# Substra/substrafl

Hardware: AMD Instinct MI355X
Metric: aggregated-param GB/s (device-resident) FedAvg reduce, N clients × M params (higher is better)
Workload: dtype f32

## Files before the change

substrafl_amd/csrc/host_pool.h:

```cpp
#pragma once

#include <algorithm>
#include <atomic>
#include <condition_variable>
#include <cstdint>
#include <cstring>
#include <deque>
#include <functional>
#include <mutex>
#include <thread>
#include <vector>

#include <pthread.h>
#include <sched.h>

namespace fedagg_host {

inline bool bind_thread(const std::vector<int>& cpus) {
  if (cpus.empty()) return true;
  cpu_set_t set;
  CPU_ZERO(&set);
  for (int c : cpus)
    if (c >= 0 && c < CPU_SETSIZE) CPU_SET(c, &set);
  return pthread_setaffinity_np(pthread_self(), sizeof(set), &set) == 0;
}

class Pool {
 public:
  explicit Pool(int n, std::vector<int> cpus = {}) : cpus_(std::move(cpus)) {
    for (int i = 0; i < n; ++i) th_.emplace_back([this] { run(); });
  }
  ~Pool() {
    {
      std::lock_guard<std::mutex> g(m_);
      stop_ = true;
    }
    cv_.notify_all();
    for (auto& t : th_) t.join();
  }
  void submit(std::function<void()> f) {
    {
      std::lock_guard<std::mutex> g(m_);
      q_.push_back(std::move(f));
    }
    cv_.notify_one();
  }
  int size() const { return (int)th_.size(); }
  const std::vector<int>& cpus() const { return cpus_; }

 private:
  void run() {
    bind_thread(cpus_);
    for (;;) {
      std::function<void()> f;
      {
        std::unique_lock<std::mutex> l(m_);
        cv_.wait(l, [this] { return stop_ || !q_.empty(); });
        if (stop_ && q_.empty()) return;
        f = std::move(q_.front());
        q_.pop_front();
      }
      f();
    }
  }
  const std::vector<int> cpus_;
  std::vector<std::thread> th_;
  std::deque<std::function<void()>> q_;
  std::mutex m_;
  std::condition_variable cv_;
  bool stop_ = false;
};

struct Done {
  std::mutex m;
  std::condition_variable cv;
  bool done = false;
  void set() {
    std::lock_guard<std::mutex> g(m);
    done = true;
    cv.notify_all();
  }
  void wait() {
    std::unique_lock<std::mutex> l(m);
    cv.wait(l, [this] { return done; });
  }
};

inline void gather_range(const void* const* ptr, const uint64_t* len, int nseg, uint64_t a, uint64_t b, char* dst) {
  uint64_t off = 0;
  for (int i = 0; i < nseg && off < b; ++i) {
    const uint64_t s0 = off, s1 = off + len[i];
    off = s1;
    const uint64_t lo = std::max(a, s0), hi = std::min(b, s1);
    if (lo >= hi) continue;
    memcpy(dst + (lo - a), static_cast<const char*>(ptr[i]) + (lo - s0), hi - lo);
  }
}

template <typename T>
inline uint64_t count_value_mismatch(const char* x, const char* r, uint64_t n) {
  uint64_t bad = 0;
  for (uint64_t i = 0; i < n; ++i) {
    T a, b;
    memcpy(&a, x + i * sizeof(T), sizeof(T));
    memcpy(&b, r + i * sizeof(T), sizeof(T));
    bad += !((a == b) || (a != a && b != b));
  }
  return bad;
}

enum { kHalfNone = 0, kHalfF16 = 1, kHalfBF16 = 2 };

inline uint64_t count_value_mismatch16(const char* x, const char* r, uint64_t n, uint16_t inf_bits) {
  uint64_t bad = 0;
  for (uint64_t i = 0; i < n; ++i) {
    uint16_t a, b;
    memcpy(&a, x + i * 2, 2);
    memcpy(&b, r + i * 2, 2);
    const uint16_t ma = a & 0x7FFF, mb = b & 0x7FFF;
    bad += !((a == b) || ((ma | mb) == 0) || (ma > inf_bits && mb > inf_bits));
  }
  return bad;
}

inline uint64_t count_mismatch_range(const void* const* x, const void* const* ref, const uint64_t* len, int nseg,
                                     uint64_t a, uint64_t b, int esz, int half = kHalfNone) {
  uint64_t off = 0, bad = 0;
  for (int i = 0; i < nseg && off < b; ++i) {
    const uint64_t s0 = off, s1 = off + len[i];
    off = s1;
    const uint64_t lo = std::max(a, s0), hi = std::min(b, s1);
    if (lo >= hi) continue;
    const char* px = static_cast<const char*>(x[i]) + (lo - s0);
    const char* pr = static_cast<const char*>(ref[i]) + (lo - s0);
    if (px == pr) continue;
    for (uint64_t u = 0; u < hi - lo; u += 4096) {
      const uint64_t n = std::min<uint64_t>(4096, hi - lo - u);
      if (!memcmp(px + u, pr + u, n)) continue;
      bad += half ? count_value_mismatch16(px + u, pr + u, n / 2, half == kHalfBF16 ? 0x7F80 : 0x7C00)
             : esz == 8 ? count_value_mismatch<double>(px + u, pr + u, n / 8)
                        : count_value_mismatch<float>(px + u, pr + u, n / 4);
    }
  }
  return bad;
}

struct Ring {
  std::vector<void*> slot;
  std::vector<bool> used;
  uint64_t chunk_bytes = 0;
  int size() const { return (int)slot.size(); }
};

inline uint64_t check_rows(Pool& pool, const void* const* h_seg, const uint64_t* seg_bytes, int nseg, int K,
                           uint64_t byte_lo, uint64_t row, int esz, int half = kHalfNone) {
  const uint64_t piece = 1ull << 20;
  const uint64_t npieces = (K >= 2 && row) ? (row + piece - 1) / piece : 0;
  std::atomic<uint64_t> bad{0};
  std::vector<Done> cdone(npieces ? npieces : 1);
  for (uint64_t p = 0; p < npieces; ++p) {
    const uint64_t a = byte_lo + p * piece, b = byte_lo + std::min(row, (p + 1) * piece);
    Done* d = &cdone[p];
    pool.submit([=, &bad] {
      uint64_t n = 0;
      for (int k = 1; k < K; ++k) n += count_mismatch_range(h_seg + (size_t)k * nseg, h_seg, seg_bytes, nseg, a, b, esz, half);
      bad.fetch_add(n, std::memory_order_relaxed);
      d->set();
    });
  }
  for (uint64_t p = 0; p < npieces; ++p) cdone[p].wait();
  return bad.load();
}

template <class Eng, class Pack, class Copy>
int ring_stage(Eng& eng, Pool& pool, Ring& ring, uint64_t units, bool two_queues, Pack pack, Copy copy) {
  const int R = ring.size();
  const bool two = two_queues && units > 1;
  std::vector<Done> done(units ? std::min<uint64_t>(units, (uint64_t)R) : 1);
  std::vector<bool> pending(done.size(), false);
  int rc = 0;
  uint64_t next_submit = 0;
  auto submit = [&](uint64_t u) {
    const int slot = (int)(u % R);
    if (ring.used[slot]) eng.wait(slot);
    ring.used[slot] = false;
    Done& d = done[slot];
    d.done = false;
    pending[slot] = true;
    char* dst = static_cast<char*>(ring.slot[slot]);
    pool.submit([=, &d] {
      pack(u, dst);
      d.set();
    });
  };
  for (; next_submit < units && next_submit + 1 < (uint64_t)R; ++next_submit) submit(next_submit);
  for (uint64_t u = 0; u < units && !rc; ++u) {
    const int slot = (int)(u % R);
    done[slot].wait();
    pending[slot] = false;
    const int q = (two && (u & 1)) ? 1 : 0;
    rc = copy(u, static_cast<const char*>(ring.slot[slot]), q);
    if (!rc) rc = eng.mark(slot, q);
    if (!rc) ring.used[slot] = true;
    if (!rc && next_submit < units) submit(next_submit++);
  }
  for (size_t i = 0; i < done.size(); ++i)
    if (pending[i]) done[i].wait();
  return rc;
}

template <class Eng>
int stage_pipeline(Eng& eng, Pool& pool, Ring& ring, const void* const* h_seg, const uint64_t* seg_bytes, int nseg,
                   int K, uint64_t byte_lo, uint64_t row, char* d_dst, uint64_t ld_bytes, bool two_queues,
                   int check_esz = 0, uint64_t* mismatches = nullptr, int check_half = kHalfNone) {
  const uint64_t cb = ring.chunk_bytes;
  const int Ks = check_esz ? 1 : K;
  const uint64_t per_row = row ? (row + cb - 1) / cb : 0;
  const int rc = ring_stage(
      eng, pool, ring, per_row * (uint64_t)Ks, two_queues,
      [=](uint64_t u, char* dst) {
        const uint64_t a = (u % per_row) * cb, b = std::min(row, a + cb);
        gather_range(h_seg + (size_t)(u / per_row) * nseg, seg_bytes, nseg, byte_lo + a, byte_lo + b, dst);
      },
      [&, per_row, cb](uint64_t u, const char* slot, int q) {
        const uint64_t a = (u % per_row) * cb;
        return eng.h2d(q, d_dst + (u / per_row) * ld_bytes + a, slot, std::min(row, a + cb) - a);
      });
  if (rc || !check_esz || K < 2) return rc;
  const uint64_t bad = check_rows(pool, h_seg, seg_bytes, nseg, K, byte_lo, row, check_esz, check_half);
  if (mismatches) *mismatches += bad;
  return 0;
}

template <class Eng>
int stage_tiled_pipeline(Eng& eng, Pool& pool, Ring& ring, const void* const* h_seg, const uint64_t* seg_bytes,
                         int nseg, int K, uint64_t row, uint64_t tb, char* d_dst, bool two_queues) {
  if (!tb || tb > ring.chunk_bytes) return -1;
  const uint64_t tiles = row ? (row + tb - 1) / tb : 0;
  const uint64_t blocks = tiles * (uint64_t)K, bpu = ring.chunk_bytes / tb;
  return ring_stage(
      eng, pool, ring, (blocks + bpu - 1) / bpu, two_queues,
      [=](uint64_t u, char* dst) {
        const uint64_t j1 = std::min(blocks, (u + 1) * bpu);
        for (uint64_t j = u * bpu; j < j1; ++j) {
          const uint64_t t = j / (uint64_t)K, a = t * tb, b = std::min(row, a + tb);
          gather_range(h_seg + (size_t)(j % (uint64_t)K) * nseg, seg_bytes, nseg, a, b, dst + (j - u * bpu) * tb);
        }
      },
      [&, blocks, bpu](uint64_t u, const char* slot, int q) {
        return eng.h2d(q, d_dst + u * bpu * tb, slot, (std::min(blocks, (u + 1) * bpu) - u * bpu) * tb);
      });
}

template <class Eng>
int stage_row_tiled_pipeline(Eng& eng, Pool& pool, Ring& ring, const void* const* h_seg, const uint64_t* seg_bytes,
                             int nseg, uint64_t row, uint64_t tb, int K, int k, char* d_dst, bool two_queues) {
  if (!tb || tb > ring.chunk_bytes || K <= 0 || k < 0 || k >= K) return -1;
  const uint64_t tiles = row ? (row + tb - 1) / tb : 0, tpu = ring.chunk_bytes / tb;
  return ring_stage(
      eng, pool, ring, (tiles + tpu - 1) / tpu, two_queues,
      [=](uint64_t u, char* dst) {
        const uint64_t a = u * tpu * tb;
        gather_range(h_seg, seg_bytes, nseg, a, std::min(row, a + tpu * tb), dst);
      },
      [&, tiles, tpu](uint64_t u, const char* slot, int q) {
        const uint64_t t0 = u * tpu, n = std::min(tiles, t0 + tpu) - t0;
        return eng.h2d_2d(q, d_dst + (t0 * (uint64_t)K + (uint64_t)k) * tb, (uint64_t)K * tb, slot, tb, tb, n);
      });
}

template <class Eng>
int fetch_pipeline(Eng& eng, Pool& pool, Ring& ring, const char* d_src, char* h_dst, uint64_t bytes) {
  const uint64_t cb = ring.chunk_bytes;
  const int R = ring.size();
  const int G = std::max(1, std::min(4, R / 2));
  const int NG = R / G;
  const uint64_t sb = cb * (uint64_t)G;
  const uint64_t units = (bytes + sb - 1) / sb;
  std::vector<Done> done(R);
  std::vector<bool> pending(R, false);
  int rc = 0;
  for (uint64_t u = 0; u < units && !rc; ++u) {
    const int g0 = (int)(u % (uint64_t)NG) * G;
    for (int i = 0; i < G; ++i)
      if (pending[g0 + i]) {
        done[g0 + i].wait();
        pending[g0 + i] = false;
      }
    const uint64_t a = u * sb, b = std::min(bytes, a + sb);
    rc = eng.d2h(ring.slot[g0], d_src + a, b - a);
    if (!rc) rc = eng.mark(g0, 0);
    if (rc) break;
    for (int i = 0; i < G; ++i) ring.used[g0 + i] = i == 0;
    for (int i = 0; i < G; ++i) {
      const uint64_t pa = a + (uint64_t)i * cb;
      if (pa >= b) break;
      const uint64_t pb = std::min(b, pa + cb);
      const int slot = g0 + i;
      done[slot].done = false;
      pending[slot] = true;
      const char* src = static_cast<const char*>(ring.slot[slot]);
      char* dst = h_dst + pa;
      Done* d = &done[slot];
      pool.submit([=, &eng] {
        eng.wait(g0);
        memcpy(dst, src, pb - pa);
        d->set();
      });
    }
  }
  for (int i = 0; i < R; ++i)
    if (pending[i]) done[i].wait();
  return rc;
}

}
```

substrafl_amd/csrc/session.hip:

```cpp

#include <hip/hip_runtime.h>

#include <algorithm>
#include <atomic>
#include <chrono>
#include <condition_variable>
#include <cstdint>
#include <cstdio>
#include <cstring>
#include <deque>
#include <functional>
#include <mutex>
#include <thread>
#include <vector>

#include <sys/syscall.h>
#include <unistd.h>

#include "fedagg_internal.h"
#include "host_pool.h"

using fedagg_host::Pool;
using fedagg_host::Ring;

namespace {

int hip_fail(const char* what, hipError_t e) {
  char buf[512];
  snprintf(buf, sizeof(buf), "%s: %s", what, hipGetErrorString(e));
  fedagg_internal::set_error(buf);
  return FEDAGG_EHIP;
}

#define HIP_TRY(call)                                     \
  do {                                                    \
    hipError_t e_ = (call);                               \
    if (e_ != hipSuccess) return hip_fail(#call, e_);     \
  } while (0)

}

struct fedagg_session {
  int device = 0;
  hipStream_t stream = nullptr;
  hipStream_t xstream = nullptr;
  hipEvent_t join_ev = nullptr;
  int copy_streams = 2;
  int threads = 8;
  uint64_t chunk_bytes = 4ull << 20;
  int slots = 12;
  void* ring_base = nullptr;
  Ring ring;
  std::vector<hipEvent_t> ring_ev;
  void* dbuf[FEDAGG_SESSION_BUFFERS] = {};
  uint64_t dbytes[FEDAGG_SESSION_BUFFERS] = {};
  hipEvent_t tev[FEDAGG_SESSION_EVENTS] = {};
  Pool* pool = nullptr;
  double last_stage_s = 0, last_fetch_s = 0;
  uint64_t fail_copy_after = 0;
  uint64_t copies = 0;
  std::vector<int> cpus;
  double phase[FEDAGG_SESSION_PHASES] = {};

  int ensure_ring() {
    if (ring.size() == slots && ring.chunk_bytes == chunk_bytes) return FEDAGG_OK;
    release_ring();
    ring.slot.assign(slots, nullptr);
    ring_ev.assign(slots, nullptr);
    ring.used.assign(slots, false);
    ring.chunk_bytes = chunk_bytes;
    hipError_t e;
    if (cpus.empty()) {
      e = hipHostMalloc(&ring_base, (size_t)slots * chunk_bytes, hipHostMallocDefault);
    } else {
      e = hipErrorUnknown;
      std::thread t([&] {
        (void)hipSetDevice(device);
        if (fedagg_host::bind_thread(cpus))
          e = hipHostMalloc(&ring_base, (size_t)slots * chunk_bytes, hipHostMallocNumaUser);
        else
          e = hipHostMalloc(&ring_base, (size_t)slots * chunk_bytes, hipHostMallocDefault);
      });
      t.join();
    }
    if (e != hipSuccess) {
      ring_base = nullptr;
      release_ring();
      return hip_fail("hipHostMalloc(staging ring)", e);
    }
    for (int i = 0; i < slots; ++i) {
      ring.slot[i] = static_cast<char*>(ring_base) + (size_t)i * chunk_bytes;
      if ((e = hipEventCreateWithFlags(&ring_ev[i], hipEventDisableTiming)) != hipSuccess) {
        ring_ev[i] = nullptr;
        release_ring();
        return hip_fail("hipEventCreate(staging ring)", e);
      }
    }
    return FEDAGG_OK;
  }
  void release_ring() {
    for (size_t i = 0; i < ring_ev.size(); ++i) {
      if (ring_ev[i]) {
        (void)hipEventSynchronize(ring_ev[i]);
        (void)hipEventDestroy(ring_ev[i]);
      }
    }
    if (ring_base) (void)hipHostFree(ring_base);
    ring_base = nullptr;
    ring.slot.clear();
    ring.used.clear();
    ring.chunk_bytes = 0;
    ring_ev.clear();
  }
  std::mutex pool_m;
  Pool& workers() {
    std::lock_guard<std::mutex> g(pool_m);
    if (!pool || pool->size() != threads || pool->cpus() != cpus) {
      delete pool;
      pool = new Pool(threads, cpus);
    }
    return *pool;
  }
};

namespace {

double now_s() {
  return std::chrono::duration<double>(std::chrono::steady_clock::now().time_since_epoch()).count();
}

struct HipEngine {
  fedagg_session* s;
  bool injected() { return s->fail_copy_after && ++s->copies >= s->fail_copy_after; }
  int h2d(int q, void* d, const void* h, uint64_t n) {
    if (injected()) return hip_fail("hipMemcpyAsync(H2D) [injected by the fail_copy_after knob]", hipErrorUnknown);
    hipError_t e = hipMemcpyAsync(d, h, n, hipMemcpyHostToDevice, q ? s->xstream : s->stream);
    return e == hipSuccess ? FEDAGG_OK : hip_fail("hipMemcpyAsync(H2D)", e);
  }
  int h2d_2d(int q, void* d, uint64_t dpitch, const void* h, uint64_t spitch, uint64_t width, uint64_t height) {
    if (injected()) return hip_fail("hipMemcpy2DAsync(H2D) [injected by the fail_copy_after knob]", hipErrorUnknown);
    hipError_t e = hipMemcpy2DAsync(d, dpitch, h, spitch, width, height, hipMemcpyHostToDevice,
                                    q ? s->xstream : s->stream);
    return e == hipSuccess ? FEDAGG_OK : hip_fail("hipMemcpy2DAsync(H2D)", e);
  }
  int d2h(void* h, const void* d, uint64_t n) {
    if (injected()) return hip_fail("hipMemcpyAsync(D2H) [injected by the fail_copy_after knob]", hipErrorUnknown);
    hipError_t e = hipMemcpyAsync(h, d, n, hipMemcpyDeviceToHost, s->stream);
    return e == hipSuccess ? FEDAGG_OK : hip_fail("hipMemcpyAsync(D2H)", e);
  }
  int mark(int slot, int q) {
    hipError_t e = hipEventRecord(s->ring_ev[slot], q ? s->xstream : s->stream);
    return e == hipSuccess ? FEDAGG_OK : hip_fail("hipEventRecord(ring)", e);
  }
  void wait(int slot) { (void)hipEventSynchronize(s->ring_ev[slot]); }
};

}

extern "C" {

fedagg_session* fedagg_session_create(int device) {
  const double t0 = now_s();
  int n = 0;
  hipError_t e = hipGetDeviceCount(&n);
  if (e != hipSuccess || n <= 0) {
    hip_fail("fedagg_session_create: no HIP device", e == hipSuccess ? hipErrorNoDevice : e);
    return nullptr;
  }
  if (device < 0 || device >= n) {
    fedagg_internal::set_error("fedagg_session_create: device index out of range");
    return nullptr;
  }
  if ((e = hipSetDevice(device)) != hipSuccess) {
    hip_fail("hipSetDevice", e);
    return nullptr;
  }
  auto* s = new fedagg_session();
  s->device = device;
  const double t1 = now_s();
  s->phase[0] = t1 - t0;
  if ((e = hipStreamCreateWithFlags(&s->stream, hipStreamNonBlocking)) != hipSuccess ||
      (e = hipStreamCreateWithFlags(&s->xstream, hipStreamNonBlocking)) != hipSuccess ||
      (e = hipEventCreateWithFlags(&s->join_ev, hipEventDisableTiming)) != hipSuccess) {
    hip_fail("fedagg_session_create: stream/event", e);
    if (s->xstream) (void)hipStreamDestroy(s->xstream);
    if (s->stream) (void)hipStreamDestroy(s->stream);
    delete s;
    return nullptr;
  }
  s->phase[1] = now_s() - t1;
  return s;
}

void fedagg_session_destroy(fedagg_session* s) {
  if (!s) return;
  (void)hipSetDevice(s->device);
  (void)hipStreamSynchronize(s->stream);
  (void)hipStreamSynchronize(s->xstream);
  s->release_ring();
  for (int i = 0; i < FEDAGG_SESSION_BUFFERS; ++i)
    if (s->dbuf[i]) (void)hipFree(s->dbuf[i]);
  for (int i = 0; i < FEDAGG_SESSION_EVENTS; ++i)
    if (s->tev[i]) (void)hipEventDestroy(s->tev[i]);
  (void)hipEventDestroy(s->join_ev);
  (void)hipStreamDestroy(s->xstream);
  (void)hipStreamDestroy(s->stream);
  delete s->pool;
  delete s;
}

void* fedagg_session_stream(fedagg_session* s) { return s ? (void*)s->stream : nullptr; }

int fedagg_session_set(fedagg_session* s, const char* key, long long value) {
  if (!s || !key) return FEDAGG_EINVAL;
  if (!strcmp(key, "threads") && value >= 1 && value <= 256) {
    s->threads = (int)value;
    if (s->slots < s->threads + 2) {
      s->release_ring();
      s->slots = s->threads + 2;
    }
  } else if (!strcmp(key, "chunk_bytes") && value >= (1 << 16)) {
    s->release_ring();
    s->chunk_bytes = (uint64_t)value;
  } else if (!strcmp(key, "copy_streams") && (value == 1 || value == 2)) {
    s->copy_streams = (int)value;
  } else if (!strcmp(key, "slots") && value >= 2 && value <= 1024) {
    s->release_ring();
    s->slots = (int)std::max<long long>(value, s->threads + 1);
  } else if (!strcmp(key, "fail_copy_after") && value >= 0) {
    s->fail_copy_after = (uint64_t)value;
    s->copies = 0;
  } else {
    fedagg_internal::set_error("fedagg_session_set: unknown key or bad value");
    return FEDAGG_EINVAL;
  }
  return FEDAGG_OK;
}

int fedagg_session_affinity(fedagg_session* s, const int* cpus, int ncpus) {
  if (!s || ncpus < 0 || (ncpus && !cpus)) {
    fedagg_internal::set_error("fedagg_session_affinity: invalid argument");
    return FEDAGG_EINVAL;
  }
  std::vector<int> v(cpus, cpus + ncpus);
  for (int c : v)
    if (c < 0 || c >= CPU_SETSIZE) {
      fedagg_internal::set_error("fedagg_session_affinity: CPU index out of range");
      return FEDAGG_EINVAL;
    }
  std::lock_guard<std::mutex> g(s->pool_m);
  if (v != s->cpus) {
    int caller = -1;
    (void)hipGetDevice(&caller);
    (void)hipSetDevice(s->device);
    s->release_ring();
    s->cpus = std::move(v);
    if (caller >= 0) (void)hipSetDevice(caller);
  }
  return FEDAGG_OK;
}

int fedagg_session_ring_node(fedagg_session* s) {
  if (!s || !s->ring_base) return -1;
  int node = -1;
  if (syscall(SYS_get_mempolicy, &node, nullptr, 0UL, s->ring_base, 3UL) != 0) return -1;
  return node;
}

int fedagg_device_pci_bus_id(int device, char* buf, int len) {
  if (!buf || len < 13) {
    fedagg_internal::set_error("fedagg_device_pci_bus_id: buffer too small");
    return FEDAGG_EINVAL;
  }
  hipError_t e = hipDeviceGetPCIBusId(buf, len, device);
  return e == hipSuccess ? FEDAGG_OK : hip_fail("hipDeviceGetPCIBusId", e);
}

int fedagg_session_buffer(fedagg_session* s, int slot, uint64_t bytes, void** d_ptr) {
  if (!s || slot < 0 || slot >= FEDAGG_SESSION_BUFFERS || !d_ptr) return FEDAGG_EINVAL;
  HIP_TRY(hipSetDevice(s->device));
  if (s->dbytes[slot] < bytes) {
    if (s->dbuf[slot]) {
      HIP_TRY(hipStreamSynchronize(s->stream));
      HIP_TRY(hipFree(s->dbuf[slot]));
      s->dbuf[slot] = nullptr;
      s->dbytes[slot] = 0;
    }
    HIP_TRY(hipMalloc(&s->dbuf[slot], bytes));
    s->dbytes[slot] = bytes;
  }
  *d_ptr = s->dbuf[slot];
  return FEDAGG_OK;
}

int fedagg_session_warm(fedagg_session* s, const uint64_t* slot_bytes, int nslots) {
  if (!s || nslots < 0 || nslots > FEDAGG_SESSION_BUFFERS || (nslots > 0 && !slot_bytes)) return FEDAGG_EINVAL;
  HIP_TRY(hipSetDevice(s->device));
  double t = now_s();
  int rc = s->ensure_ring();
  if (rc) return rc;
  s->phase[2] = now_s() - t;
  t = now_s();
  (void)s->workers();
  s->phase[3] = now_s() - t;
  t = now_s();
  void* probe = nullptr;
  for (int i = 0; i < nslots; ++i) {
    if (!slot_bytes[i]) continue;
    void* d = nullptr;
    rc = fedagg_session_buffer(s, i, slot_bytes[i], &d);
    if (rc) return rc;
    if (!probe && slot_bytes[i] >= 4096) probe = d;
  }
  if (!probe) {
    rc = fedagg_session_buffer(s, FEDAGG_SESSION_BUFFERS - 1, 4096, &probe);
    if (rc) return rc;
  }
  s->phase[4] = now_s() - t;
  t = now_s();
  HIP_TRY(hipMemsetAsync(probe, 0, 4096, s->stream));
  rc = fedagg_read_probe_f32(static_cast<const float*>(probe), 512, static_cast<float*>(probe) + 512, 1,
                             (void*)s->stream);
  if (rc) return rc;
  HIP_TRY(hipStreamSynchronize(s->stream));
  s->phase[5] = now_s() - t;
  return FEDAGG_OK;
}

int fedagg_session_stage(fedagg_session* s, void* d_dst, uint64_t ld_bytes, int K, int nseg,
                         const void* const* h_seg, const uint64_t* seg_bytes) {
  if (nseg < 0 || (nseg > 0 && !seg_bytes)) return FEDAGG_EINVAL;
  uint64_t row = 0;
  for (int i = 0; i < nseg; ++i) row += seg_bytes[i];
  return fedagg_session_stage_range(s, d_dst, ld_bytes, K, nseg, h_seg, seg_bytes, 0, row);
}

namespace {

int stage_prepare(fedagg_session* s, void* d_dst, uint64_t ld_bytes, int K, int nseg, const void* const* h_seg,
                  const uint64_t* seg_bytes, uint64_t byte_lo, uint64_t byte_hi, uint64_t* row_out) {
  if (!s || !d_dst || K <= 0 || nseg < 0 || (nseg > 0 && (!h_seg || !seg_bytes)) || byte_hi < byte_lo)
    return FEDAGG_EINVAL;
  HIP_TRY(hipSetDevice(s->device));
  int rc = s->ensure_ring();
  if (rc) return rc;
  uint64_t full = 0;
  for (int i = 0; i < nseg; ++i) full += seg_bytes[i];
  if (byte_hi > full) {
    fedagg_internal::set_error("fedagg_session_stage_range: byte range beyond the row");
    return FEDAGG_EINVAL;
  }
  const uint64_t row = byte_hi - byte_lo;
  if (row > ld_bytes) {
    fedagg_internal::set_error("fedagg_session_stage: segments exceed the row stride");
    return FEDAGG_EINVAL;
  }
  for (int k = 0; k < K; ++k)
    for (int i = 0; i < nseg; ++i)
      if (!h_seg[(size_t)k * nseg + i] && seg_bytes[i]) {
        fedagg_internal::set_error("fedagg_session_stage: NULL host segment");
        return FEDAGG_EINVAL;
      }
  *row_out = row;
  return FEDAGG_OK;
}

}
}
namespace {
template <class Run>
int stage_run_with(fedagg_session* s, Run run) {
  const double t0 = now_s();
  const bool two = s->copy_streams > 1;
  if (two) {
    HIP_TRY(hipEventRecord(s->join_ev, s->stream));
    HIP_TRY(hipStreamWaitEvent(s->xstream, s->join_ev, 0));
  }
  HipEngine eng{s};
  int rc = run(eng, two);
  if (two) {
    hipError_t e = hipEventRecord(s->join_ev, s->xstream);
    if (e == hipSuccess) e = hipStreamWaitEvent(s->stream, s->join_ev, 0);
    if (e != hipSuccess && !rc) rc = hip_fail("fedagg_session_stage: join of the copy queues", e);
  }
  s->last_stage_s = now_s() - t0;
  return rc;
}

int stage_run(fedagg_session* s, void* d_dst, uint64_t ld_bytes, int K, int nseg, const void* const* h_seg,
              const uint64_t* seg_bytes, uint64_t byte_lo, uint64_t row, int check_esz, uint64_t* mismatches,
              int check_half = fedagg_host::kHalfNone) {
  return stage_run_with(s, [&](HipEngine& eng, bool two) {
    return fedagg_host::stage_pipeline(eng, s->workers(), s->ring, h_seg, seg_bytes, nseg, K, byte_lo, row,
                                       static_cast<char*>(d_dst), ld_bytes, two, check_esz, mismatches, check_half);
  });
}

}

extern "C" {

int fedagg_session_stage_range(fedagg_session* s, void* d_dst, uint64_t ld_bytes, int K, int nseg,
                               const void* const* h_seg, const uint64_t* seg_bytes, uint64_t byte_lo,
                               uint64_t byte_hi) {
  uint64_t row = 0;
  int rc = stage_prepare(s, d_dst, ld_bytes, K, nseg, h_seg, seg_bytes, byte_lo, byte_hi, &row);
  if (rc) return rc;
  return stage_run(s, d_dst, ld_bytes, K, nseg, h_seg, seg_bytes, byte_lo, row, 0, nullptr);
}

int fedagg_session_stage_tiled(fedagg_session* s, void* d_dst, uint64_t tile_bytes, int K, int nseg,
                               const void* const* h_seg, const uint64_t* seg_bytes) {
  if (nseg < 0 || (nseg > 0 && !seg_bytes)) return FEDAGG_EINVAL;
  uint64_t full = 0, row = 0;
  for (int i = 0; i < nseg; ++i) full += seg_bytes[i];
  int rc = stage_prepare(s, d_dst, full, K, nseg, h_seg, seg_bytes, 0, full, &row);
  if (rc) return rc;
  if (!tile_bytes || tile_bytes % 16 || tile_bytes > s->chunk_bytes) {
    fedagg_internal::set_error("fedagg_session_stage_tiled: tile_bytes must be a multiple of 16 and <= chunk_bytes");
    return FEDAGG_EINVAL;
  }
  return stage_run_with(s, [&](HipEngine& eng, bool two) {
    return fedagg_host::stage_tiled_pipeline(eng, s->workers(), s->ring, h_seg, seg_bytes, nseg, K, row, tile_bytes,
                                             static_cast<char*>(d_dst), two);
  });
}

int fedagg_session_stage_tiled_row(fedagg_session* s, void* d_dst, uint64_t tile_bytes, int K, int k, int nseg,
                                   const void* const* h_seg, const uint64_t* seg_bytes) {
  if (nseg < 0 || (nseg > 0 && !seg_bytes)) return FEDAGG_EINVAL;
  if (K <= 0 || k < 0 || k >= K) {
    fedagg_internal::set_error("fedagg_session_stage_tiled_row: need 0 <= k < K");
    return FEDAGG_EINVAL;
  }
  uint64_t full = 0, row = 0;
  for (int i = 0; i < nseg; ++i) full += seg_bytes[i];
  int rc = stage_prepare(s, d_dst, full, 1, nseg, h_seg, seg_bytes, 0, full, &row);
  if (rc) return rc;
  if (!tile_bytes || tile_bytes % 16 || tile_bytes > s->chunk_bytes) {
    fedagg_internal::set_error("fedagg_session_stage_tiled_row: tile_bytes must be a multiple of 16 and <= chunk_bytes");
    return FEDAGG_EINVAL;
  }
  return stage_run_with(s, [&](HipEngine& eng, bool two) {
    return fedagg_host::stage_row_tiled_pipeline(eng, s->workers(), s->ring, h_seg, seg_bytes, nseg, row, tile_bytes,
                                                 K, k, static_cast<char*>(d_dst), two);
  });
}

int fedagg_session_stage_check(fedagg_session* s, void* d_dst, int K, int nseg, const void* const* h_seg,
                               const uint64_t* seg_bytes, uint64_t byte_lo, uint64_t byte_hi, int kind,
                               uint64_t* mismatches) {
  if (!mismatches || (kind != FEDAGG_F32 && kind != FEDAGG_F64 && kind != FEDAGG_F16 && kind != FEDAGG_BF16)) {
    fedagg_internal::set_error(
        "fedagg_session_stage_check: kind must be FEDAGG_F16, FEDAGG_BF16, FEDAGG_F32 or FEDAGG_F64");
    return FEDAGG_EINVAL;
  }
  const int esz = kind == FEDAGG_F64 ? 8 : kind == FEDAGG_F32 ? 4 : 2;
  const int half = kind == FEDAGG_F16    ? fedagg_host::kHalfF16
                   : kind == FEDAGG_BF16 ? fedagg_host::kHalfBF16
                                         : fedagg_host::kHalfNone;
  for (int i = 0; i < nseg && seg_bytes; ++i)
    if (seg_bytes[i] % esz) {
      fedagg_internal::set_error("fedagg_session_stage_check: segment not a whole number of elements");
      return FEDAGG_EINVAL;
    }
  if (byte_lo % esz || byte_hi % esz) {
    fedagg_internal::set_error("fedagg_session_stage_check: byte range not element-aligned");
    return FEDAGG_EINVAL;
  }
  *mismatches = 0;
  if (!d_dst) {
    if (!s || K <= 0 || nseg < 0 || (nseg > 0 && (!h_seg || !seg_bytes)) || byte_hi < byte_lo) return FEDAGG_EINVAL;
    uint64_t full = 0;
    for (int i = 0; i < nseg; ++i) full += seg_bytes[i];
    for (int k = 0; k < K; ++k)
      for (int i = 0; i < nseg; ++i)
        if (!h_seg[(size_t)k * nseg + i] && seg_bytes[i]) {
          fedagg_internal::set_error("fedagg_session_stage_check: NULL host segment");
          return FEDAGG_EINVAL;
        }
    if (byte_hi > full) {
      fedagg_internal::set_error("fedagg_session_stage_check: byte range beyond the row");
      return FEDAGG_EINVAL;
    }
    *mismatches = fedagg_host::check_rows(s->workers(), h_seg, seg_bytes, nseg, K, byte_lo, byte_hi - byte_lo, esz, half);
    return FEDAGG_OK;
  }
  uint64_t row = 0;
  int rc = stage_prepare(s, d_dst, byte_hi - byte_lo, K, nseg, h_seg, seg_bytes, byte_lo, byte_hi, &row);
  if (rc) return rc;
  return stage_run(s, d_dst, row, K, nseg, h_seg, seg_bytes, byte_lo, row, esz, mismatches, half);
}

int fedagg_session_fetch(fedagg_session* s, const void* d_src, void* h_dst, uint64_t bytes) {
  if (!s || !d_src || (!h_dst && bytes)) return FEDAGG_EINVAL;
  const double t0 = now_s();
  HIP_TRY(hipSetDevice(s->device));
  int rc = s->ensure_ring();
  if (rc) return rc;
  HipEngine eng{s};
  rc = fedagg_host::fetch_pipeline(eng, s->workers(), s->ring, static_cast<const char*>(d_src),
                                   static_cast<char*>(h_dst), bytes);
  s->last_fetch_s = now_s() - t0;
  return rc;
}

int fedagg_session_event_record(fedagg_session* s, int ev) {
  if (!s || ev < 0 || ev >= FEDAGG_SESSION_EVENTS) return FEDAGG_EINVAL;
  HIP_TRY(hipSetDevice(s->device));
  if (!s->tev[ev]) HIP_TRY(hipEventCreate(&s->tev[ev]));
  HIP_TRY(hipEventRecord(s->tev[ev], s->stream));
  return FEDAGG_OK;
}

int fedagg_session_event_elapsed(fedagg_session* s, int ev0, int ev1, float* ms) {
  if (!s || !ms || ev0 < 0 || ev1 < 0 || ev0 >= FEDAGG_SESSION_EVENTS || ev1 >= FEDAGG_SESSION_EVENTS ||
      !s->tev[ev0] || !s->tev[ev1])
    return FEDAGG_EINVAL;
  HIP_TRY(hipEventSynchronize(s->tev[ev1]));
  HIP_TRY(hipEventElapsedTime(ms, s->tev[ev0], s->tev[ev1]));
  return FEDAGG_OK;
}

int fedagg_session_activate(fedagg_session* s) {
  if (!s) return FEDAGG_EINVAL;
  HIP_TRY(hipSetDevice(s->device));
  return FEDAGG_OK;
}

int fedagg_device_count(void) {
  int n = 0;
  if (hipGetDeviceCount(&n) != hipSuccess) return 0;
  return n;
}

int fedagg_device_get(int* device_out) {
  if (!device_out) return FEDAGG_EINVAL;
  HIP_TRY(hipGetDevice(device_out));
  return FEDAGG_OK;
}

int fedagg_device_set(int device) {
  HIP_TRY(hipSetDevice(device));
  return FEDAGG_OK;
}

int fedagg_device_memory(int device, uint64_t* free_bytes, uint64_t* total_bytes) {
  if (!free_bytes || !total_bytes) return FEDAGG_EINVAL;
  HIP_TRY(hipSetDevice(device));
  size_t f = 0, t = 0;
  HIP_TRY(hipMemGetInfo(&f, &t));
  *free_bytes = f;
  *total_bytes = t;
  return FEDAGG_OK;
}

int fedagg_session_memset(fedagg_session* s, void* d, int value, uint64_t bytes) {
  if (!s || !d) return FEDAGG_EINVAL;
  HIP_TRY(hipSetDevice(s->device));
  HIP_TRY(hipMemsetAsync(d, value, bytes, s->stream));
  return FEDAGG_OK;
}

int fedagg_session_copy_d2d(fedagg_session* s, void* d_dst, const void* d_src, uint64_t bytes) {
  if (!s || (bytes && (!d_dst || !d_src))) return FEDAGG_EINVAL;
  if (!bytes) return FEDAGG_OK;
  HIP_TRY(hipSetDevice(s->device));
  HIP_TRY(hipMemcpyAsync(d_dst, d_src, bytes, hipMemcpyDeviceToDevice, s->stream));
  return FEDAGG_OK;
}

int fedagg_session_sync(fedagg_session* s) {
  if (!s) return FEDAGG_EINVAL;
  HIP_TRY(hipSetDevice(s->device));
  HIP_TRY(hipStreamSynchronize(s->stream));
  return FEDAGG_OK;
}

int fedagg_session_phases(fedagg_session* s, double* out, int n) {
  if (!s || n < 0 || (n && !out)) return FEDAGG_EINVAL;
  for (int i = 0; i < n && i < FEDAGG_SESSION_PHASES; ++i) out[i] = s->phase[i];
  return FEDAGG_OK;
}

int fedagg_session_timing(fedagg_session* s, double* stage_s, double* fetch_s) {
  if (!s) return FEDAGG_EINVAL;
  if (stage_s) *stage_s = s->last_stage_s;
  if (fetch_s) *fetch_s = s->last_fetch_s;
  return FEDAGG_OK;
}

}
```

substrafl_amd/runtime.py:

```python

from __future__ import annotations

import ctypes
import os
import threading
from typing import Dict, List, Optional, Sequence

import numpy as np

from . import _native

KIND_CODE = {
    np.dtype(np.float16): 0,
    np.dtype(np.float32): 1,
    np.dtype(np.float64): 2,
    np.dtype(np.int8): 3,
    np.dtype(np.int16): 4,
    np.dtype(np.int32): 5,
    np.dtype(np.int64): 6,
    np.dtype(np.uint8): 7,
    np.dtype(np.uint16): 8,
    np.dtype(np.uint32): 9,
    np.dtype(np.uint64): 10,
    np.dtype(np.bool_): 11,
}


def kind_code(dtype) -> int:
    d = np.dtype(dtype)
    if d not in KIND_CODE:
        raise NotImplementedError(f"no device conversion for dtype {d}")
    return KIND_CODE[d]


class Session:

    def __init__(self, device: int = 0, threads: Optional[int] = None):
        self.lib = _native.load()
        h = self.lib.fedagg_session_create(int(device))
        if not h:
            raise _native.NativeLibraryError(
                "cannot open a HIP session on device %d: %s (the aggregation engine runs on MI355X only, "
                "no CPU fallback)" % (device, self.lib.fedagg_last_error().decode(errors="replace"))
            )
        self._h = ctypes.c_void_p(h)
        self.device = int(device)
        self._held: Dict[int, int] = {}
        self._ptr: Dict[int, int] = {}
        self._gen: Dict[int, int] = {}
        self.stream = int(self.lib.fedagg_session_stream(self._h) or 0)
        nthreads = threads or int(os.environ.get("FEDAGG_PACK_THREADS", "0")) or min(16, os.cpu_count() or 1)
        self.set("threads", nthreads)
        if os.environ.get("FEDAGG_COPY_STREAMS"):
            self.set("copy_streams", int(os.environ["FEDAGG_COPY_STREAMS"]))

    def close(self) -> None:
        if getattr(self, "_h", None):
            self.lib.fedagg_session_destroy(self._h)
            self._h = None

    def __del__(self):
        try:
            self.close()
        except Exception:
            pass

    def __reduce__(self):
        raise TypeError("a Session holds a GPU context and cannot be pickled")

    def set(self, key: str, value: int) -> None:
        _native.check(self.lib.fedagg_session_set(self._h, key.encode(), int(value)), f"session_set({key})")

    def affinity(self, cpus: Optional[Sequence[int]]) -> None:
        cpus = [int(c) for c in (cpus or [])]
        arr = (ctypes.c_int * max(1, len(cpus)))(*cpus)
        _native.check(self.lib.fedagg_session_affinity(self._h, arr, len(cpus)), "session_affinity")

    def ring_node(self) -> int:
        return int(self.lib.fedagg_session_ring_node(self._h))

    def warm(self, slot_bytes: Dict[int, int]) -> None:
        n = _native.FEDAGG_SESSION_BUFFERS
        arr = (ctypes.c_uint64 * n)(*[int(slot_bytes.get(i, 0)) for i in range(n)])
        _native.check(self.lib.fedagg_session_warm(self._h, arr, n), "session_warm")

    def held_bytes(self, slots: Optional[Sequence[int]] = None) -> int:
        if slots is None:
            return sum(self._held.values())
        return sum(self._held.get(int(k), 0) for k in set(slots))

    def buffer(self, slot: int, nbytes: int) -> int:
        slot = int(slot)
        need = max(16, int(nbytes))
        grew = need > self._held.get(slot, 0)
        self._held[slot] = max(self._held.get(slot, 0), need)
        p = ctypes.c_void_p()
        _native.check(self.lib.fedagg_session_buffer(self._h, slot, need, ctypes.byref(p)), "session_buffer")
        if grew or self._ptr.get(slot) != int(p.value):
            self._ptr[slot] = int(p.value)
            self._gen[slot] = self._gen.get(slot, 0) + 1
        return int(p.value)

    def _slot_of(self, d: int) -> Optional[int]:
        for slot, base in self._ptr.items():
            if base <= d < base + self._held.get(slot, 0):
                return slot
        return None

    def _bump(self, d: int) -> None:
        slot = self._slot_of(int(d))
        if slot is not None:
            self._gen[slot] = self._gen.get(slot, 0) + 1

    def generation(self, slot: int) -> int:
        return self._gen.get(int(slot), 0)

    def stage(self, d_dst: int, ld_bytes: int, rows: Sequence[Sequence[np.ndarray]],
              byte_range: Optional[tuple] = None) -> None:
        K = len(rows)
        nseg, ptrs, sizes, keep = _segments(rows)
        self._bump(d_dst)
        if byte_range is None:
            _native.check(self.lib.fedagg_session_stage(self._h, ctypes.c_void_p(d_dst), int(ld_bytes), K, nseg,
                                                        ptrs, sizes), "session_stage")
        else:
            lo, hi = (int(v) for v in byte_range)
            _native.check(self.lib.fedagg_session_stage_range(self._h, ctypes.c_void_p(d_dst), int(ld_bytes), K,
                                                              nseg, ptrs, sizes, lo, hi), "session_stage_range")

    def stage_tiled(self, d_dst: int, tile_bytes: int, rows: Sequence[Sequence[np.ndarray]]) -> None:
        nseg, ptrs, sizes, keep = _segments(rows)
        self._bump(d_dst)
        _native.check(self.lib.fedagg_session_stage_tiled(self._h, ctypes.c_void_p(d_dst), int(tile_bytes), len(rows),
                                                          nseg, ptrs, sizes), "session_stage_tiled")

    def stage_tiled_row(self, d_dst: int, tile_bytes: int, K: int, k: int, row: Sequence[np.ndarray]) -> None:
        nseg, ptrs, sizes, keep = _segments([row])
        self._bump(d_dst)
        _native.check(self.lib.fedagg_session_stage_tiled_row(self._h, ctypes.c_void_p(d_dst), int(tile_bytes), int(K),
                                                              int(k), nseg, ptrs, sizes), "session_stage_tiled_row")

    def stage_check(self, d_dst: int, rows: Sequence[Sequence[np.ndarray]], dtype,
                    byte_range: Optional[tuple] = None) -> int:
        from .wire import BF16

        dtype = np.dtype(dtype)
        kind = {np.dtype(np.float16): _native.FEDAGG_F16, BF16: _native.FEDAGG_BF16,
                np.dtype(np.float32): _native.FEDAGG_F32, np.dtype(np.float64): _native.FEDAGG_F64}[dtype]
        nseg, ptrs, sizes, keep = _segments(rows)
        for row in rows:
            for a in row:
                if a.dtype != dtype:
                    raise ValueError("stage_check: every array must have the checked dtype")
        lo, hi = (0, sum(int(sizes[i]) for i in range(nseg))) if byte_range is None else byte_range
        if d_dst:
            self._bump(d_dst)
        mism = ctypes.c_uint64(0)
        _native.check(self.lib.fedagg_session_stage_check(self._h, ctypes.c_void_p(d_dst), len(rows), nseg, ptrs,
                                                          sizes, int(lo), int(hi), kind, ctypes.byref(mism)),
                      "session_stage_check")
        return int(mism.value)

    def check(self, rows: Sequence[Sequence[np.ndarray]], dtype) -> int:
        return self.stage_check(0, rows, dtype)

    def event_record(self, ev: int) -> None:
        _native.check(self.lib.fedagg_session_event_record(self._h, int(ev)), "session_event_record")

    def event_elapsed_ms(self, ev0: int, ev1: int) -> float:
        ms = ctypes.c_float()
        _native.check(self.lib.fedagg_session_event_elapsed(self._h, int(ev0), int(ev1), ctypes.byref(ms)),
                      "session_event_elapsed")
        return float(ms.value)

    def activate(self) -> None:
        _native.check(self.lib.fedagg_session_activate(self._h), "session_activate")

    def fetch(self, d_src: int, out: np.ndarray) -> np.ndarray:
        if not out.flags.c_contiguous:
            raise ValueError("fetch destination must be C-contiguous")
        _native.check(self.lib.fedagg_session_fetch(self._h, ctypes.c_void_p(d_src),
                                                    ctypes.c_void_p(out.ctypes.data), out.nbytes), "session_fetch")
        return out

    def memset(self, d: int, value: int, nbytes: int) -> None:
        self._bump(d)
        _native.check(self.lib.fedagg_session_memset(self._h, ctypes.c_void_p(d), int(value), int(nbytes)),
                      "session_memset")

    def copy_d2d(self, d_dst: int, d_src: int, nbytes: int) -> None:
        self._bump(d_dst)
        _native.check(self.lib.fedagg_session_copy_d2d(self._h, ctypes.c_void_p(d_dst), ctypes.c_void_p(d_src),
                                                       int(nbytes)), "session_copy_d2d")

    def sync(self) -> None:
        _native.check(self.lib.fedagg_session_sync(self._h), "session_sync")

    def timing(self) -> Dict[str, float]:
        a, b = ctypes.c_double(), ctypes.c_double()
        self.lib.fedagg_session_timing(self._h, ctypes.byref(a), ctypes.byref(b))
        return {"stage_s": a.value, "fetch_s": b.value}

    PHASES = ("hip_init_s", "streams_s", "ring_s", "pool_s", "buffers_s", "code_object_s")

    def phases(self) -> Dict[str, float]:
        n = _native.FEDAGG_SESSION_PHASES
        out = (ctypes.c_double * n)()
        _native.check(self.lib.fedagg_session_phases(self._h, out, n), "session_phases")
        return {k: round(float(v), 6) for k, v in zip(self.PHASES, out)}

    def cast(self, d_in: int, in_dtype, d_out: int, out_dtype, n: int) -> None:
        self._bump(d_out)
        _native.check(self.lib.fedagg_cast(ctypes.c_void_p(d_in), kind_code(in_dtype), ctypes.c_void_p(d_out),
                                           kind_code(out_dtype), int(n), ctypes.c_void_p(self.stream)), "cast")

    def scale_cast(self, d_in: int, in_dtype, w: float, d_out: int, out_dtype, n: int) -> None:
        self._bump(d_out)
        _native.check(self.lib.fedagg_scale_cast(ctypes.c_void_p(d_in), kind_code(in_dtype), float(w),
                                                 ctypes.c_void_p(d_out), kind_code(out_dtype), int(n),
                                                 ctypes.c_void_p(self.stream)), "scale_cast")


def _segments(rows: Sequence[Sequence[np.ndarray]]):
    K = len(rows)
    nseg = len(rows[0]) if K else 0
    keep: List[np.ndarray] = []
    ptrs = (ctypes.c_void_p * max(1, K * nseg))()
    sizes = (ctypes.c_uint64 * max(1, nseg))()
    for k, row in enumerate(rows):
        if len(row) != nseg:
            raise ValueError("every client row needs the same segments")
        for i, a in enumerate(row):
            a = np.ascontiguousarray(a)
            keep.append(a)
            ptrs[k * nseg + i] = a.ctypes.data if a.nbytes else None
            if k == 0:
                sizes[i] = a.nbytes
            elif a.nbytes != sizes[i]:
                raise ValueError("segment sizes differ between clients")
    return nseg, ptrs, sizes, keep


_device_locks: Dict[int, threading.RLock] = {}


def device_lock(device: int) -> threading.RLock:
    with _lock:
        lk = _device_locks.get(int(device))
        if lk is None:
            lk = _device_locks[int(device)] = threading.RLock()
        return lk


_host_cache: Dict[tuple, dict] = {}
_host_lock = threading.Lock()
HOST_POOL_DEPTH = 64
HOST_POOL_BYTES = 16 << 30
HOST_POOL_IDLE = 2


def reusable_host_array(n: int, dtype, tag: str) -> np.ndarray:
    import sys

    key = (tag, np.dtype(dtype))
    with _host_lock:
        site = _host_cache.setdefault(key, {"tick": 0, "pool": []})
        site["tick"] += 1
        tick, pool = site["tick"], site["pool"]
        out = None
        for i in range(len(pool) - 1, -1, -1):
            buf = pool[i][0]
            if buf.size >= n and sys.getrefcount(buf) <= 3:
                ent = pool.pop(i)
                ent[1] = tick
                pool.append(ent)
                buf.flags.writeable = True
                out = buf[:n]
                break
        buf = None
        if out is None:
            out = np.empty(n, dtype=key[1])
            pool.append([out, tick])
        idle = HOST_POOL_IDLE * max(2, len(pool))
        keep = []
        for ent in pool:
            b = ent[0]
            if tick - ent[1] > idle and b is not out and b is not getattr(out, "base", None) \
                    and sys.getrefcount(b) <= 3:
                continue
            keep.append(ent)
        b = None
        pool[:] = keep
        while len(pool) > 1 and (len(pool) > HOST_POOL_DEPTH or sum(e[0].nbytes for e in pool) > HOST_POOL_BYTES):
            pool.pop(0)
        return out


def drop_host_pools() -> None:
    with _host_lock:
        _host_cache.clear()


def device_pci_bus_id(device: int) -> str:
    lib = _native.load()
    buf = ctypes.create_string_buffer(64)
    _native.check(lib.fedagg_device_pci_bus_id(int(device), buf, len(buf)), "device_pci_bus_id")
    return buf.value.decode().lower()


def device_memory(device: int) -> tuple:
    lib = _native.load()
    f, t = ctypes.c_uint64(), ctypes.c_uint64()
    _native.check(lib.fedagg_device_memory(int(device), ctypes.byref(f), ctypes.byref(t)), "device_memory")
    return int(f.value), int(t.value)


_sessions: Dict[int, Session] = {}
_lock = threading.Lock()
_warming: Dict[int, threading.Thread] = {}
_warm_errors: Dict[int, BaseException] = {}
warm_times: Dict[int, tuple] = {}
warm_phases: Dict[int, dict] = {}


def session(device: int = 0) -> Session:
    t = _warming.get(device)
    if t is not None and t is not threading.current_thread():
        t.join()
    with _lock:
        s = _sessions.get(device)
        if s is None:
            s = _sessions[device] = Session(device)
        return s


def prewarm(device: int = 0, slot_bytes: Optional[Dict[int, int]] = None) -> threading.Thread:
    with _lock:
        t = _warming.get(device)
        if t is not None:
            return t

        def run():
            import time

            t0 = time.perf_counter()
            ph: Dict[str, object] = {}
            try:
                _native.load()
                t1 = time.perf_counter()
                ph["library_load_s"] = round(t1 - t0, 6)
                with _lock:
                    created = device not in _sessions
                s = session(device)
                ph["session_s"] = round(time.perf_counter() - t1, 6)
                ph["created_by_prewarm"] = created
                s.warm(slot_bytes or {})
                ph.update(s.phases())
            except BaseException as e:
                _warm_errors[device] = e
            t_end = time.perf_counter()
            ph["total_s"] = round(t_end - t0, 6)
            warm_phases[device] = ph
            warm_times[device] = (t0, t_end)

        t = threading.Thread(target=run, name=f"fedagg-prewarm-{device}", daemon=True)
        _warming[device] = t
    t.start()
    return t
```

Baseline: 7039.

## Coalesce contiguous ring slots into grouped H2D copies and retune staging defaults

The ring staging loop now packs up to G contiguous pinned slots as one group and issues a single larger hipMemcpyAsync per group instead of one per chunk. This is meant to cut per-copy launch and event overhead. Defaults change to one copy stream, a group of eight and 24 slots, and a copy_group knob plus an environment variable are added. Grouping needs contiguous slots, reduces per-slot overlap granularity, and drops the second copy queue by default.

Result: no change. 7039 (-0.0%).

```diff
diff --git a/substrafl_amd/csrc/host_pool.h b/substrafl_amd/csrc/host_pool.h
--- a/substrafl_amd/csrc/host_pool.h
+++ b/substrafl_amd/csrc/host_pool.h
@@ -149,8 +149,24 @@
   std::vector<void*> slot;
   std::vector<bool> used;
   uint64_t chunk_bytes = 0;
+  int group = 1;
   int size() const { return (int)slot.size(); }
 };
+
+inline int stage_group(const Ring& ring) {
+  const int R = ring.size();
+  int G = std::max(1, std::min(ring.group, R / 2));
+  for (int i = 0; G > 1 && i + 1 < R; ++i)
+    if (static_cast<const char*>(ring.slot[i + 1]) != static_cast<const char*>(ring.slot[i]) + ring.chunk_bytes) G = 1;
+  return G;
+}
+
+template <class Eng>
+auto note_chunks(Eng& eng, uint64_t n, int) -> decltype(eng.chunks(n), void()) {
+  eng.chunks(n);
+}
+template <class Eng>
+void note_chunks(Eng&, uint64_t, long) {}
 
 inline uint64_t check_rows(Pool& pool, const void* const* h_seg, const uint64_t* seg_bytes, int nseg, int K,
                            uint64_t byte_lo, uint64_t row, int esz, int half = kHalfNone) {
@@ -173,38 +189,54 @@
 }
 
 template <class Eng, class Pack, class Copy>
-int ring_stage(Eng& eng, Pool& pool, Ring& ring, uint64_t units, bool two_queues, Pack pack, Copy copy) {
-  const int R = ring.size();
+int ring_stage(Eng& eng, Pool& pool, Ring& ring, uint64_t units, uint64_t run, uint64_t unit_bytes, bool two_queues,
+               Pack pack, Copy copy) {
+  const int R = ring.size(), G = stage_group(ring);
+  const uint64_t NG = (uint64_t)(R / G);
   const bool two = two_queues && units > 1;
-  std::vector<Done> done(units ? std::min<uint64_t>(units, (uint64_t)R) : 1);
-  std::vector<bool> pending(done.size(), false);
+  std::vector<Done> done(R);
+  std::vector<bool> pending(R, false);
   int rc = 0;
-  uint64_t next_submit = 0;
-  auto submit = [&](uint64_t u) {
-    const int slot = (int)(u % R);
-    if (ring.used[slot]) eng.wait(slot);
-    ring.used[slot] = false;
-    Done& d = done[slot];
-    d.done = false;
-    pending[slot] = true;
-    char* dst = static_cast<char*>(ring.slot[slot]);
-    pool.submit([=, &d] {
-      pack(u, dst);
-      d.set();
-    });
+  auto group_len = [&](uint64_t u0) { return std::min({(uint64_t)G, run - u0 % run, units - u0}); };
+  uint64_t next_unit = 0, next_group = 0;
+  auto submit = [&] {
+    const int g0 = (int)(next_group % NG) * G;
+    for (int i = 0; i < G; ++i) {
+      if (ring.used[g0 + i]) eng.wait(g0 + i);
+      ring.used[g0 + i] = false;
+    }
+    const uint64_t n = group_len(next_unit);
+    for (uint64_t i = 0; i < n; ++i) {
+      Done& d = done[g0 + i];
+      d.done = false;
+      pending[g0 + i] = true;
+      const uint64_t u = next_unit + i;
+      char* dst = static_cast<char*>(ring.slot[g0]) + i * unit_bytes;
+      pool.submit([=, &d] {
+        pack(u, dst);
+        d.set();
+      });
+    }
+    next_unit += n;
+    ++next_group;
   };
-  for (; next_submit < units && next_submit + 1 < (uint64_t)R; ++next_submit) submit(next_submit);
-  for (uint64_t u = 0; u < units && !rc; ++u) {
-    const int slot = (int)(u % R);
-    done[slot].wait();
-    pending[slot] = false;
-    const int q = (two && (u & 1)) ? 1 : 0;
-    rc = copy(u, static_cast<const char*>(ring.slot[slot]), q);
-    if (!rc) rc = eng.mark(slot, q);
-    if (!rc) ring.used[slot] = true;
-    if (!rc && next_submit < units) submit(next_submit++);
-  }
-  for (size_t i = 0; i < done.size(); ++i)
+  while (next_unit < units && next_group + 1 < NG) submit();
+  for (uint64_t u = 0, j = 0; u < units && !rc; ++j) {
+    const int g0 = (int)(j % NG) * G;
+    const uint64_t n = group_len(u);
+    for (uint64_t i = 0; i < n; ++i) {
+      done[g0 + i].wait();
+      pending[g0 + i] = false;
+    }
+    const int q = (two && (j & 1)) ? 1 : 0;
+    if (n > 1) note_chunks(eng, n - 1, 0);
+    rc = copy(u, n, static_cast<const char*>(ring.slot[g0]), q);
+    if (!rc) rc = eng.mark(g0, q);
+    if (!rc) ring.used[g0] = true;
+    if (!rc && next_unit < units) submit();
+    u += n;
+  }
+  for (int i = 0; i < R; ++i)
     if (pending[i]) done[i].wait();
   return rc;
 }
@@ -217,14 +249,14 @@
   const int Ks = check_esz ? 1 : K;
   const uint64_t per_row = row ? (row + cb - 1) / cb : 0;
   const int rc = ring_stage(
-      eng, pool, ring, per_row * (uint64_t)Ks, two_queues,
+      eng, pool, ring, per_row * (uint64_t)Ks, std::max<uint64_t>(1, per_row), cb, two_queues,
       [=](uint64_t u, char* dst) {
         const uint64_t a = (u % per_row) * cb, b = std::min(row, a + cb);
         gather_range(h_seg + (size_t)(u / per_row) * nseg, seg_bytes, nseg, byte_lo + a, byte_lo + b, dst);
       },
-      [&, per_row, cb](uint64_t u, const char* slot, int q) {
+      [&, per_row, cb](uint64_t u, uint64_t n, const char* src, int q) {
         const uint64_t a = (u % per_row) * cb;
-        return eng.h2d(q, d_dst + (u / per_row) * ld_bytes + a, slot, std::min(row, a + cb) - a);
+        return eng.h2d(q, d_dst + (u / per_row) * ld_bytes + a, src, std::min(row, a + n * cb) - a);
       });
   if (rc || !check_esz || K < 2) return rc;
   const uint64_t bad = check_rows(pool, h_seg, seg_bytes, nseg, K, byte_lo, row, check_esz, check_half);
@@ -237,9 +269,9 @@
                          int nseg, int K, uint64_t row, uint64_t tb, char* d_dst, bool two_queues) {
   if (!tb || tb > ring.chunk_bytes) return -1;
   const uint64_t tiles = row ? (row + tb - 1) / tb : 0;
-  const uint64_t blocks = tiles * (uint64_t)K, bpu = ring.chunk_bytes / tb;
+  const uint64_t blocks = tiles * (uint64_t)K, bpu = ring.chunk_bytes / tb, units = (blocks + bpu - 1) / bpu;
   return ring_stage(
-      eng, pool, ring, (blocks + bpu - 1) / bpu, two_queues,
+      eng, pool, ring, units, std::max<uint64_t>(1, units), bpu * tb, two_queues,
       [=](uint64_t u, char* dst) {
         const uint64_t j1 = std::min(blocks, (u + 1) * bpu);
         for (uint64_t j = u * bpu; j < j1; ++j) {
@@ -247,8 +279,8 @@
           gather_range(h_seg + (size_t)(j % (uint64_t)K) * nseg, seg_bytes, nseg, a, b, dst + (j - u * bpu) * tb);
         }
       },
-      [&, blocks, bpu](uint64_t u, const char* slot, int q) {
-        return eng.h2d(q, d_dst + u * bpu * tb, slot, (std::min(blocks, (u + 1) * bpu) - u * bpu) * tb);
+      [&, blocks, bpu](uint64_t u, uint64_t n, const char* src, int q) {
+        return eng.h2d(q, d_dst + u * bpu * tb, src, (std::min(blocks, (u + n) * bpu) - u * bpu) * tb);
       });
 }
 
@@ -256,16 +288,16 @@
 int stage_row_tiled_pipeline(Eng& eng, Pool& pool, Ring& ring, const void* const* h_seg, const uint64_t* seg_bytes,
                              int nseg, uint64_t row, uint64_t tb, int K, int k, char* d_dst, bool two_queues) {
   if (!tb || tb > ring.chunk_bytes || K <= 0 || k < 0 || k >= K) return -1;
-  const uint64_t tiles = row ? (row + tb - 1) / tb : 0, tpu = ring.chunk_bytes / tb;
+  const uint64_t tiles = row ? (row + tb - 1) / tb : 0, tpu = ring.chunk_bytes / tb, units = (tiles + tpu - 1) / tpu;
   return ring_stage(
-      eng, pool, ring, (tiles + tpu - 1) / tpu, two_queues,
+      eng, pool, ring, units, std::max<uint64_t>(1, units), tpu * tb, two_queues,
       [=](uint64_t u, char* dst) {
         const uint64_t a = u * tpu * tb;
         gather_range(h_seg, seg_bytes, nseg, a, std::min(row, a + tpu * tb), dst);
       },
-      [&, tiles, tpu](uint64_t u, const char* slot, int q) {
-        const uint64_t t0 = u * tpu, n = std::min(tiles, t0 + tpu) - t0;
-        return eng.h2d_2d(q, d_dst + (t0 * (uint64_t)K + (uint64_t)k) * tb, (uint64_t)K * tb, slot, tb, tb, n);
+      [&, tiles, tpu](uint64_t u, uint64_t n, const char* src, int q) {
+        const uint64_t t0 = u * tpu, nt = std::min(tiles, t0 + n * tpu) - t0;
+        return eng.h2d_2d(q, d_dst + (t0 * (uint64_t)K + (uint64_t)k) * tb, (uint64_t)K * tb, src, tb, tb, nt);
       });
 }
 
diff --git a/substrafl_amd/csrc/session.hip b/substrafl_amd/csrc/session.hip
--- a/substrafl_amd/csrc/session.hip
+++ b/substrafl_amd/csrc/session.hip
@@ -45,10 +45,11 @@
   hipStream_t stream = nullptr;
   hipStream_t xstream = nullptr;
   hipEvent_t join_ev = nullptr;
-  int copy_streams = 2;
+  int copy_streams = 1;
+  int copy_group = 8;
   int threads = 8;
   uint64_t chunk_bytes = 4ull << 20;
-  int slots = 12;
+  int slots = 24;
   void* ring_base = nullptr;
   Ring ring;
   std::vector<hipEvent_t> ring_ev;
@@ -69,6 +70,7 @@
     ring_ev.assign(slots, nullptr);
     ring.used.assign(slots, false);
     ring.chunk_bytes = chunk_bytes;
+    ring.group = copy_group;
     hipError_t e;
     if (cpus.empty()) {
       e = hipHostMalloc(&ring_base, (size_t)slots * chunk_bytes, hipHostMallocDefault);
@@ -132,6 +134,9 @@
 struct HipEngine {
   fedagg_session* s;
   bool injected() { return s->fail_copy_after && ++s->copies >= s->fail_copy_after; }
+  void chunks(uint64_t n) {
+    if (s->fail_copy_after) s->copies += n;
+  }
   int h2d(int q, void* d, const void* h, uint64_t n) {
     if (injected()) return hip_fail("hipMemcpyAsync(H2D) [injected by the fail_copy_after knob]", hipErrorUnknown);
     hipError_t e = hipMemcpyAsync(d, h, n, hipMemcpyHostToDevice, q ? s->xstream : s->stream);
@@ -224,6 +229,9 @@
     s->chunk_bytes = (uint64_t)value;
   } else if (!strcmp(key, "copy_streams") && (value == 1 || value == 2)) {
     s->copy_streams = (int)value;
+  } else if (!strcmp(key, "copy_group") && value >= 1 && value <= 64) {
+    s->release_ring();
+    s->copy_group = (int)value;
   } else if (!strcmp(key, "slots") && value >= 2 && value <= 1024) {
     s->release_ring();
     s->slots = (int)std::max<long long>(value, s->threads + 1);
diff --git a/substrafl_amd/runtime.py b/substrafl_amd/runtime.py
--- a/substrafl_amd/runtime.py
+++ b/substrafl_amd/runtime.py
@@ -53,6 +53,8 @@
         self.set("threads", nthreads)
         if os.environ.get("FEDAGG_COPY_STREAMS"):
             self.set("copy_streams", int(os.environ["FEDAGG_COPY_STREAMS"]))
+        if os.environ.get("FEDAGG_COPY_GROUP"):
+            self.set("copy_group", int(os.environ["FEDAGG_COPY_GROUP"]))
 
     def close(self) -> None:
         if getattr(self, "_h", None):
```
